# Terascale-All-sensing-Research-Studio/MOV-SLAM

Hardware: AMD Instinct MI355X
Metric: local-BA iterations/sec (50 KF x 20k MapPoint window) (higher is better)
Workload: dtype f64; 1 GPU; LocalBundleAdjustment 50 KF + 10 fixed x 20000 MapPoints, E=110510 mono edges, Huber on, 10 LM iterations (cfg3, seed 1003); one window per GPU; parallelism=1 window

## Files before the change

### mov-slam_amd/csrc/coarse_level.h

```cpp
#pragma once
#include <hip/hip_runtime.h>

#include <type_traits>

#include "device_math.h"
#include "device_types.h"
#include "handoff.h"

namespace movba {

#ifndef MOVBA_COARSE_EXTRAPOLATE
#define MOVBA_COARSE_EXTRAPOLATE 1
#endif

template <int kT, int kNC, int kPA>
__device__ __forceinline__ void coarse_build(const DevWindow &w, const PcgParams &pp, int trial, double lambda, double *sm, bool extrapolate)
{
    double *Ac = sm;
    double *gj = Ac + kNC * kNC;
    int &s_bad = *reinterpret_cast<int *>(gj + 9 * kNC + 2);
    const int tid = threadIdx.x;
    const int nf = w.nfree;
#ifdef MOVBA_CLOCK_STAMP
    unsigned long long cst_last = __builtin_amdgcn_s_memtime();
#define COARSE_STAMP(k) do { const unsigned long long _t = __builtin_amdgcn_s_memtime(); if (tid == 0) w.ctrl->dbg_seg2[k] += _t - cst_last; cst_last = _t; } while (0)
#else
#define COARSE_STAMP(k) do { } while (0)
#endif
    const double *part = w.part, *part_ = part;
    double *blocks = w.blocks_c;
    if (tid == 0) s_bad = 0;
    for (int idx = tid; idx < kNC * kNC; idx += kT) Ac[idx] = 0.0;

    const int ndiag = nf * 36;
    for (int idx = tid; idx < w.n_multi * 36; idx += kT) {
        const int m = idx / 36, k = idx - m * 36, pr = w.multi_pairs[m];
        double sacc = 0.0;
        for (int itx = w.pair_item_start[pr]; itx < w.pair_item_start[pr + 1]; ++itx) sacc += part[(size_t)itx * kPartStride + k];
        blocks[pr * 36 + k] = -sacc;
    }
    for (int base = tid; base < ndiag; base += 4 * kT) {
        int k[4], hu[4], i0[4], i1[4];
        double s[4] = { 0, 0, 0, 0 }, hp[4] = { 0, 0, 0, 0 };
        int nmax = 0;
#pragma unroll
        for (int m = 0; m < 4; ++m) {
            const int idx = min(base + m * kT, ndiag - 1);
            const int pr = idx / 36;
            k[m] = idx - pr * 36;
            const int a = k[m] / 6, b = k[m] - a * 6;
            hu[m] = 42 + (a <= b ? ut6(a, b) : ut6(b, a));
            i0[m] = w.pair_item_start[pr]; i1[m] = w.pair_item_start[pr + 1];
            nmax = max(nmax, i1[m] - i0[m]);
        }
        for (int o = 0; o < nmax; o += 6) {
            double sv[4][6], hv[4][6];
#pragma unroll
            for (int m = 0; m < 4; ++m)
#pragma unroll
                for (int u = 0; u < 6; ++u) {
                    const double *src = part + (size_t)min(i0[m] + o + u, i1[m] - 1) * kPartStride;
                    sv[m][u] = src[k[m]]; hv[m][u] = src[hu[m]];
                }
#pragma unroll
            for (int m = 0; m < 4; ++m)
#pragma unroll
                for (int u = 0; u < 6; ++u) { const bool in = i0[m] + o + u < i1[m]; s[m] += in ? sv[m][u] : 0.0; hp[m] += in ? hv[m][u] : 0.0; }
        }
#pragma unroll
        for (int m = 0; m < 4; ++m) {
            const int idx = base + m * kT;
            if (idx < ndiag) blocks[idx] = (hp[m] + ((k[m] % 7 == 0) ? lambda : 0.0)) - s[m];
        }
    }
    __syncthreads();
    COARSE_STAMP(2);
    double *aggc = gj;
    if (tid < kNC / kPA) {
        const int g0 = pp.wave_row0[tid], g1 = pp.wave_row0[tid + 1];
        aggc[tid] = g0 + 0.5 * (g1 - g0 - 1); aggc[kNC / kPA + tid] = 1.0 / fmax(1.0, 0.5 * (g1 - g0));
    }
    int *tent = reinterpret_cast<int *>(gj + 9 * kNC + 8), *tij = tent + w.cblk_ptr[w.n_cblk];
    for (int q = tid; q < w.cblk_ptr[w.n_cblk]; q += kT) { tent[q] = w.cblk_ent[q]; tij[q] = w.cblk_ij[q]; }
    __syncthreads();
    const int nw = w.n_cblk * 6;
    const bool split = 2 * nw <= kT;
    auto walk = [&](int cb, int a, int part, double (&s00)[6], double (&s01)[6], double (&s10)[6], double (&s11)[6]) {
        const int g = w.cblk_g[cb], h = w.cblk_h[cb];
        const double cg = aggc[g], ch = aggc[h], ig = aggc[kNC / kPA + g], ih = aggc[kNC / kPA + h];
        int t0 = w.cblk_ptr[cb], t1 = w.cblk_ptr[cb + 1];
        if (split) {
            const int n = t1 - t0, front = min(n, (((n + 1) >> 1) + 7) & ~7);
            if (part == 0) t1 = t0 + front; else t0 += front;
        }
#pragma unroll
        for (int m = 0; m < 6; ++m) s00[m] = s01[m] = s10[m] = s11[m] = 0.0;
        for (int t = t0; t < t1; t += 8) {
            int pk[8], ij[8];
            double v[8][6];
#pragma unroll
            for (int u = 0; u < 8; ++u) { const int tt = min(t + u, t1 - 1); pk[u] = tent[tt]; ij[u] = tij[tt]; }
#pragma unroll
            for (int u = 0; u < 8; ++u) {
                const int e = pk[u];
                const double *src = (e & 1) ? part_ + (size_t)(e >> 2) * kPartStride : blocks + (size_t)(e >> 2) * 36;
                const int o0 = (e & 2) ? a : a * 6, st = (e & 2) ? 6 : 1;
#pragma unroll
                for (int m = 0; m < 6; ++m) v[u][m] = src[o0 + st * m];
            }
#pragma unroll
            for (int u = 0; u < 8; ++u) {
                const bool in = t + u < t1;
                const double sgn = in ? ((pk[u] & 1) ? -1.0 : 1.0) : 0.0;
                const double pi = ((ij[u] >> 16) - cg) * ig, pj = ((ij[u] & 0xffff) - ch) * ih;
#pragma unroll
                for (int m = 0; m < 6; ++m) {
                    const double x = sgn * v[u][m];
                    s00[m] += x; s01[m] += pj * x; s10[m] += pi * x; s11[m] += pi * pj * x;
                }
            }
        }
        return Ac + (g * kPA + a) * kNC + h * kPA;
    };
    if (split) {
        const bool active = tid < 2 * nw;
        const int half = tid >= nw, wi = tid - half * nw;
        double s00[6], s01[6], s10[6], s11[6];
        double *dst = nullptr;
        if (active) dst = walk(wi / 6, wi - (wi / 6) * 6, half, s00, s01, s10, s11);
        if (active && !half) {
#pragma unroll
            for (int m = 0; m < 6; ++m) { dst[m] = s00[m]; dst[6 + m] = s01[m]; dst[6 * kNC + m] = s10[m]; dst[6 * kNC + 6 + m] = s11[m]; }
        }
        __syncthreads();
        if (active && half) {
#pragma unroll
            for (int m = 0; m < 6; ++m) { dst[m] += s00[m]; dst[6 + m] += s01[m]; dst[6 * kNC + m] += s10[m]; dst[6 * kNC + 6 + m] += s11[m]; }
        }
    } else {
        for (int wi = tid; wi < nw; wi += kT) {
            double s00[6], s01[6], s10[6], s11[6];
            double *dst = walk(wi / 6, wi - (wi / 6) * 6, 0, s00, s01, s10, s11);
#pragma unroll
            for (int m = 0; m < 6; ++m) { dst[m] = s00[m]; dst[6 + m] = s01[m]; dst[6 * kNC + m] = s10[m]; dst[6 * kNC + 6 + m] = s11[m]; }
        }
    }
    __syncthreads();
    if (tid < kNC) {
        const int g = tid / kPA, d = (tid - g * kPA) / 6, nrows = pp.wave_row0[g + 1] - pp.wave_row0[g];
        if (nrows == 0 || (d == 1 && nrows < 2)) {
            for (int j = 0; j < kNC; ++j) { Ac[tid * kNC + j] = 0.0; Ac[j * kNC + tid] = 0.0; }
        }
    }
    __syncthreads();
    if (tid < kNC) {
        const int g = tid / kPA, d = (tid - g * kPA) / 6, nrows = pp.wave_row0[g + 1] - pp.wave_row0[g];
        if (nrows == 0 || (d == 1 && nrows < 2)) Ac[tid * kNC + tid] = 1.0;
    }
    __syncthreads();
    if (extrapolate) {
        double *prev = w.ac_prev;
        const double lam_prev = prev[kNC * kNC], trial_prev = prev[kNC * kNC + 1];
        double gamma = 0.0;
        if (trial >= 1 && trial_prev == (double)(trial - 1) && lambda != lam_prev && MOVBA_COARSE_EXTRAPOLATE) {
            gamma = (lambda * (1.0 / 3.0) - lambda) / (lambda - lam_prev);
            gamma = fmin(fmax(gamma, -1.0), 1.0 / 3.0);
            if (!isfinite(gamma)) gamma = 0.0;
        }
        constexpr int kPer = kNC * kNC / kT;
        static_assert(kPer * kT == kNC * kNC, "one pass");
        double pv[kPer];
#pragma unroll
        for (int u = 0; u < kPer; ++u) pv[u] = prev[tid + u * kT];
        __syncthreads();
#pragma unroll
        for (int u = 0; u < kPer; ++u) {
            const double a = Ac[tid + u * kT];
            prev[tid + u * kT] = a;
            if (gamma != 0.0) Ac[tid + u * kT] = a + gamma * (a - pv[u]);
        }
        if (tid == 0) { prev[kNC * kNC] = lambda; prev[kNC * kNC + 1] = (double)trial; }
        __syncthreads();
    }

    COARSE_STAMP(3);
    static_assert(kNC == 96 && kT == 512, "tile layout written for 96 x 96 on 512 threads");
    double *dsc = gj + 8 * kNC + 2;
    double *pvs = gj + 8 * kNC;
    if (tid < kNC) { const double d = Ac[tid * kNC + tid]; dsc[tid] = (d > 0.0 && isfinite(d)) ? rsqrt(d) : 0.0; if (!(d > 0.0) || !isfinite(d)) s_bad = 1; }
    __syncthreads();
    const int rg = tid >> 4, cg = tid & 15;
    double t[3][6];
#pragma unroll
    for (int r = 0; r < 3; ++r)
#pragma unroll
        for (int q = 0; q < 6; ++q) t[r][q] = Ac[(3 * rg + r) * kNC + 6 * cg + q] * dsc[3 * rg + r] * dsc[6 * cg + q];
    unsigned live = 0;
    for (int q = 0; q < kNC / 6; ++q) {
        const int nrows = pp.wave_row0[(q >> 1) + 1] - pp.wave_row0[q >> 1];
        if (!(nrows == 0 || ((q & 1) && nrows < 2))) live |= 1u << q;
    }
    __syncthreads();
    auto publish = [&](auto Ctag, int gq, int buf) {
        constexpr int C = decltype(Ctag)::value;
        constexpr int lr0 = C % 3, lr1 = (C + 1) % 3;
        const int rg0 = 2 * gq + C / 3, rg1 = 2 * gq + (C + 1) / 3;
        double *R1 = gj + buf * 4 * kNC, *C1 = R1 + kNC, *R2 = C1 + kNC, *C2 = R2 + kNC;
        if (rg == rg0) {
#pragma unroll
            for (int q = 0; q < 6; ++q) R1[6 * cg + q] = t[lr0][q] + ((cg == gq && q == C) ? 1.0 : 0.0);
        }
        if (rg == rg1) {
#pragma unroll
            for (int q = 0; q < 6; ++q) R2[6 * cg + q] = t[lr1][q];
        }
        if (cg == gq) {
#pragma unroll
            for (int r = 0; r < 3; ++r) { C1[3 * rg + r] = t[r][C] - ((rg == rg0 && r == lr0) ? 1.0 : 0.0); C2[3 * rg + r] = t[r][C + 1]; }
        }
        if (rg == rg0 && cg == gq) pvs[buf] = t[lr0][C];
    };
    int kk = live ? __builtin_ctz(live) : kNC / 6;
    if (kk < kNC / 6) publish(std::integral_constant<int, 0>{}, kk, 0);
    __syncthreads();
    bool bad = s_bad != 0;
    int buf = 0;
    auto pair_step = [&](auto Ctag, int gq) -> bool {
        constexpr int C = decltype(Ctag)::value;
        constexpr int lr1 = (C + 1) % 3;
        const int k = 6 * gq + C, rg1 = 2 * gq + (C + 1) / 3;
        const double *R1 = gj + buf * 4 * kNC, *C1 = R1 + kNC, *R2 = C1 + kNC, *C2 = R2 + kNC;
        const double p1 = pvs[buf];
        const double o12 = R1[k + 1], o21 = C1[k + 1], q22 = R2[k + 1];
        double r1[6], r2[6], c1[3], c2[3];
#pragma unroll
        for (int q = 0; q < 6; ++q) { r1[q] = R1[6 * cg + q]; r2[q] = R2[6 * cg + q]; }
#pragma unroll
        for (int r = 0; r < 3; ++r) { c1[r] = C1[3 * rg + r]; c2[r] = C2[3 * rg + r]; }
        if (!(p1 > 0.0) || !isfinite(p1)) return false;
        double ip1 = __builtin_amdgcn_rcp(p1);
        ip1 = ip1 * (2.0 - p1 * ip1);
        ip1 = ip1 * (2.0 - p1 * ip1);
        const double s12 = o12 * ip1;
        const double p2 = q22 - o21 * s12;
        if (!(p2 > 0.0) || !isfinite(p2)) return false;
        double ip2 = __builtin_amdgcn_rcp(p2);
        ip2 = ip2 * (2.0 - p2 * ip2);
        ip2 = ip2 * (2.0 - p2 * ip2);
#pragma unroll
        for (int q = 0; q < 6; ++q) {
            r1[q] *= ip1;
            r2[q] = ((r2[q] - o21 * r1[q]) + ((cg == gq && q == C + 1) ? 1.0 : 0.0)) * ip2;
        }
#pragma unroll
        for (int r = 0; r < 3; ++r) c2[r] = (c2[r] - c1[r] * s12) - ((rg == rg1 && r == lr1) ? 1.0 : 0.0);
#pragma unroll
        for (int r = 0; r < 3; ++r)
#pragma unroll
            for (int q = 0; q < 6; ++q) { t[r][q] -= c1[r] * r1[q]; t[r][q] -= c2[r] * r2[q]; }
        return true;
    };
    while (kk < kNC / 6 && !bad) {
        const unsigned later = kk < 31 ? (live & ~((2u << kk) - 1u)) : 0u;
        const int next = later ? __builtin_ctz(later) : kNC / 6;
        if (!pair_step(std::integral_constant<int, 0>{}, kk)) { bad = true; break; }
        publish(std::integral_constant<int, 2>{}, kk, buf ^ 1);
        __syncthreads(); buf ^= 1;
        if (!pair_step(std::integral_constant<int, 2>{}, kk)) { bad = true; break; }
        publish(std::integral_constant<int, 4>{}, kk, buf ^ 1);
        __syncthreads(); buf ^= 1;
        if (!pair_step(std::integral_constant<int, 4>{}, kk)) { bad = true; break; }
        if (next < kNC / 6) publish(std::integral_constant<int, 0>{}, next, buf ^ 1);
        __syncthreads(); buf ^= 1;
        kk = next;
    }
    if (bad && tid == 0) s_bad = 1;
    __syncthreads();
    COARSE_STAMP(4);
    float *dst = w.aci + (size_t)(trial & 1) * kNC * kNC;
#pragma unroll
    for (int r = 0; r < 3; ++r)
#pragma unroll
        for (int q = 0; q < 6; ++q) dst[(3 * rg + r) * kNC + 6 * cg + q] = (float)(t[r][q] * dsc[3 * rg + r] * dsc[6 * cg + q]);
    __syncthreads();
    if (tid == 0) w.aci_tag[trial & 1] = s_bad ? -1 : trial;
    COARSE_STAMP(5);
}

}
```

Before: 9360 LM iterations/s.

## Block the coarse Gauss-Jordan inverse into 16-wide panels with f64 MFMA updates

Replaces the 2-column-at-a-time Gauss-Jordan inversion of the 96x96 coarse matrix, which issued a barrier after every pivot pair, with a panel-blocked version. Each 16-column panel is factored in registers by three waves using readlane broadcasts. The trailing update then runs as 16x16 tiles through f64 MFMA, reading double-buffered padded panel images stored in place of A_c. This cuts the barrier count from about 48 to about 12 and moves the rank updates onto matrix cores. In exchange it adds shared-memory image traffic, and the panel liveness test and sign conventions have to stay numerically equivalent to the old version.

```diff
diff --git a/mov-slam_amd/csrc/coarse_level.h b/mov-slam_amd/csrc/coarse_level.h
--- a/mov-slam_amd/csrc/coarse_level.h
+++ b/mov-slam_amd/csrc/coarse_level.h
@@ -1,7 +1,5 @@
 #pragma once
 #include <hip/hip_runtime.h>
-
-#include <type_traits>
 
 #include "device_math.h"
 #include "device_types.h"
@@ -185,103 +183,128 @@
 
     COARSE_STAMP(3);
     static_assert(kNC == 96 && kT == 512, "tile layout written for 96 x 96 on 512 threads");
+    constexpr int kPB = 16, kNP = kNC / kPB, kPL = kPB + 1;
+    constexpr int kTilesPerWave = (kNP * kNP + kT / 64 - 1) / (kT / 64);
+    static_assert(2 * 2 * kNC * kPL <= kNC * kNC, "two pairs of panel images in the place of A_c");
+    typedef double dbl4 __attribute__((ext_vector_type(4)));
     double *dsc = gj + 8 * kNC + 2;
-    double *pvs = gj + 8 * kNC;
     if (tid < kNC) { const double d = Ac[tid * kNC + tid]; dsc[tid] = (d > 0.0 && isfinite(d)) ? rsqrt(d) : 0.0; if (!(d > 0.0) || !isfinite(d)) s_bad = 1; }
     __syncthreads();
-    const int rg = tid >> 4, cg = tid & 15;
-    double t[3][6];
-#pragma unroll
-    for (int r = 0; r < 3; ++r)
-#pragma unroll
-        for (int q = 0; q < 6; ++q) t[r][q] = Ac[(3 * rg + r) * kNC + 6 * cg + q] * dsc[3 * rg + r] * dsc[6 * cg + q];
+    const int ln = tid & 63, li = ln & 15, lk = ln >> 4;
+    const int wv = __builtin_amdgcn_readfirstlane(tid >> 6);
+    dbl4 acc[kTilesPerWave];
+#pragma unroll
+    for (int u = 0; u < kTilesPerWave; ++u) {
+        const int T = wv + 8 * u, rb = T / kNP, cb = T - rb * kNP;
+        acc[u] = dbl4{ 0.0, 0.0, 0.0, 0.0 };
+        if (T < kNP * kNP) {
+#pragma unroll
+            for (int v = 0; v < 4; ++v) {
+                const int r = kPB * rb + lk + 4 * v, q = kPB * cb + li;
+                acc[u][v] = Ac[r * kNC + q] * dsc[r] * dsc[q];
+            }
+        }
+    }
     unsigned live = 0;
     for (int q = 0; q < kNC / 6; ++q) {
         const int nrows = pp.wave_row0[(q >> 1) + 1] - pp.wave_row0[q >> 1];
         if (!(nrows == 0 || ((q & 1) && nrows < 2))) live |= 1u << q;
     }
-    __syncthreads();
-    auto publish = [&](auto Ctag, int gq, int buf) {
-        constexpr int C = decltype(Ctag)::value;
-        constexpr int lr0 = C % 3, lr1 = (C + 1) % 3;
-        const int rg0 = 2 * gq + C / 3, rg1 = 2 * gq + (C + 1) / 3;
-        double *R1 = gj + buf * 4 * kNC, *C1 = R1 + kNC, *R2 = C1 + kNC, *C2 = R2 + kNC;
-        if (rg == rg0) {
-#pragma unroll
-            for (int q = 0; q < 6; ++q) R1[6 * cg + q] = t[lr0][q] + ((cg == gq && q == C) ? 1.0 : 0.0);
-        }
-        if (rg == rg1) {
-#pragma unroll
-            for (int q = 0; q < 6; ++q) R2[6 * cg + q] = t[lr1][q];
-        }
-        if (cg == gq) {
-#pragma unroll
-            for (int r = 0; r < 3; ++r) { C1[3 * rg + r] = t[r][C] - ((rg == rg0 && r == lr0) ? 1.0 : 0.0); C2[3 * rg + r] = t[r][C + 1]; }
-        }
-        if (rg == rg0 && cg == gq) pvs[buf] = t[lr0][C];
+    unsigned plive = 0;
+    for (int P = 0; P < kNP; ++P) {
+        const int q0 = (kPB * P) / 6, q1 = (kPB * P + kPB - 1) / 6;
+        if ((live >> q0) & ((2u << (q1 - q0)) - 1u)) plive |= 1u << P;
+    }
+    __syncthreads();
+    if (s_bad) plive = 0;
+    auto image = [&](int buf) { return Ac + buf * 2 * kNC * kPL; };
+    auto store_tile = [&](double *img, int rb, const dbl4 &a) {
+#pragma unroll
+        for (int v = 0; v < 4; ++v) img[(kPB * rb + lk + 4 * v) * kPL + li] = a[v];
     };
-    int kk = live ? __builtin_ctz(live) : kNC / 6;
-    if (kk < kNC / 6) publish(std::integral_constant<int, 0>{}, kk, 0);
-    __syncthreads();
-    bool bad = s_bad != 0;
-    int buf = 0;
-    auto pair_step = [&](auto Ctag, int gq) -> bool {
-        constexpr int C = decltype(Ctag)::value;
-        constexpr int lr1 = (C + 1) % 3;
-        const int k = 6 * gq + C, rg1 = 2 * gq + (C + 1) / 3;
-        const double *R1 = gj + buf * 4 * kNC, *C1 = R1 + kNC, *R2 = C1 + kNC, *C2 = R2 + kNC;
-        const double p1 = pvs[buf];
-        const double o12 = R1[k + 1], o21 = C1[k + 1], q22 = R2[k + 1];
-        double r1[6], r2[6], c1[3], c2[3];
-#pragma unroll
-        for (int q = 0; q < 6; ++q) { r1[q] = R1[6 * cg + q]; r2[q] = R2[6 * cg + q]; }
-#pragma unroll
-        for (int r = 0; r < 3; ++r) { c1[r] = C1[3 * rg + r]; c2[r] = C2[3 * rg + r]; }
-        if (!(p1 > 0.0) || !isfinite(p1)) return false;
-        double ip1 = __builtin_amdgcn_rcp(p1);
-        ip1 = ip1 * (2.0 - p1 * ip1);
-        ip1 = ip1 * (2.0 - p1 * ip1);
-        const double s12 = o12 * ip1;
-        const double p2 = q22 - o21 * s12;
-        if (!(p2 > 0.0) || !isfinite(p2)) return false;
-        double ip2 = __builtin_amdgcn_rcp(p2);
-        ip2 = ip2 * (2.0 - p2 * ip2);
-        ip2 = ip2 * (2.0 - p2 * ip2);
-#pragma unroll
-        for (int q = 0; q < 6; ++q) {
-            r1[q] *= ip1;
-            r2[q] = ((r2[q] - o21 * r1[q]) + ((cg == gq && q == C + 1) ? 1.0 : 0.0)) * ip2;
-        }
-#pragma unroll
-        for (int r = 0; r < 3; ++r) c2[r] = (c2[r] - c1[r] * s12) - ((rg == rg1 && r == lr1) ? 1.0 : 0.0);
-#pragma unroll
-        for (int r = 0; r < 3; ++r)
-#pragma unroll
-            for (int q = 0; q < 6; ++q) { t[r][q] -= c1[r] * r1[q]; t[r][q] -= c2[r] * r2[q]; }
-        return true;
+    auto chain = [&](int P, const double *O, double *N) {
+        const int c0 = kPB * P;
+        const bool real = ln < 32;
+        const int i = real ? 32 * wv + ln : c0 + li;
+        double p[kPB];
+#pragma unroll
+        for (int c = 0; c < kPB; ++c) p[c] = O[i * kPL + c];
+        bool bad = false;
+#pragma unroll
+        for (int k = 0; k < kPB; ++k) {
+            double s[kPB];
+#pragma unroll
+            for (int c = 0; c < kPB; ++c) s[c] = readlane_f64(p[c], 32 + k);
+            const double piv = s[k];
+            bad |= !(piv > 0.0 && piv < __builtin_inf());
+            const double r0 = __builtin_amdgcn_rcp(piv);
+            const double e = __builtin_fma(-piv, r0, 1.0);
+            const double t = __builtin_fma(e, e, e);
+            const double ip = __builtin_fma(r0, t, r0);
+            const double g = (p[k] - (i == c0 + k ? 1.0 : 0.0)) * ip;
+            s[k] += 1.0;
+#pragma unroll
+            for (int c = 0; c < kPB; ++c) p[c] -= g * s[c];
+        }
+        if (real) {
+#pragma unroll
+            for (int c = 0; c < kPB; ++c) N[i * kPL + c] = p[c];
+        }
+        if (bad && ln == 0) s_bad = 1;
     };
-    while (kk < kNC / 6 && !bad) {
-        const unsigned later = kk < 31 ? (live & ~((2u << kk) - 1u)) : 0u;
-        const int next = later ? __builtin_ctz(later) : kNC / 6;
-        if (!pair_step(std::integral_constant<int, 0>{}, kk)) { bad = true; break; }
-        publish(std::integral_constant<int, 2>{}, kk, buf ^ 1);
-        __syncthreads(); buf ^= 1;
-        if (!pair_step(std::integral_constant<int, 2>{}, kk)) { bad = true; break; }
-        publish(std::integral_constant<int, 4>{}, kk, buf ^ 1);
-        __syncthreads(); buf ^= 1;
-        if (!pair_step(std::integral_constant<int, 4>{}, kk)) { bad = true; break; }
-        if (next < kNC / 6) publish(std::integral_constant<int, 0>{}, next, buf ^ 1);
-        __syncthreads(); buf ^= 1;
-        kk = next;
-    }
-    if (bad && tid == 0) s_bad = 1;
-    __syncthreads();
+    int P = plive ? __builtin_ctz(plive) : kNP, buf = 0;
+    if (P < kNP) {
+#pragma unroll
+        for (int u = 0; u < kTilesPerWave; ++u) {
+            const int T = wv + 8 * u, rb = T / kNP, cb = T - rb * kNP;
+            if (T < kNP * kNP && cb == P) store_tile(image(0), rb, acc[u]);
+        }
+    }
+    __syncthreads();
+    while (P < kNP) {
+        const unsigned later = plive & ~((2u << P) - 1u);
+        const int next = later ? __builtin_ctz(later) : kNP;
+        const double *O = image(buf), *N = O + kNC * kPL;
+        if (wv < 3) chain(P, O, image(buf) + kNC * kPL);
+        __syncthreads();
+#pragma unroll
+        for (int u = 0; u < kTilesPerWave; ++u) {
+            const int T = wv + 8 * u, rb = T / kNP, cb = T - rb * kNP;
+            if (T >= kNP * kNP) continue;
+            if (cb == P) {
+#pragma unroll
+                for (int v = 0; v < 4; ++v) acc[u][v] = N[(kPB * rb + lk + 4 * v) * kPL + li];
+            } else if (rb == P) {
+                const double sgn = cb < P ? 1.0 : -1.0;
+#pragma unroll
+                for (int v = 0; v < 4; ++v) acc[u][v] = sgn * N[(kPB * cb + li) * kPL + lk + 4 * v];
+            } else {
+                const double sgn = cb > P ? 1.0 : -1.0;
+                const double *ap = N + (kPB * rb + li) * kPL + lk, *bp = O + (kPB * cb + li) * kPL + lk;
+                double a[kPB / 4], b[kPB / 4];
+#pragma unroll
+                for (int q = 0; q < kPB / 4; ++q) { a[q] = ap[4 * q]; b[q] = sgn * bp[4 * q]; }
+#pragma unroll
+                for (int q = 0; q < kPB / 4; ++q) acc[u] = __builtin_amdgcn_mfma_f64_16x16x4f64(a[q], b[q], acc[u], 0, 0, 0);
+            }
+            if (cb == next) store_tile(image(buf ^ 1), rb, acc[u]);
+        }
+        __syncthreads();
+        buf ^= 1; P = next;
+    }
     COARSE_STAMP(4);
     float *dst = w.aci + (size_t)(trial & 1) * kNC * kNC;
 #pragma unroll
-    for (int r = 0; r < 3; ++r)
-#pragma unroll
-        for (int q = 0; q < 6; ++q) dst[(3 * rg + r) * kNC + 6 * cg + q] = (float)(t[r][q] * dsc[3 * rg + r] * dsc[6 * cg + q]);
+    for (int u = 0; u < kTilesPerWave; ++u) {
+        const int T = wv + 8 * u, rb = T / kNP, cb = T - rb * kNP;
+        if (T < kNP * kNP) {
+#pragma unroll
+            for (int v = 0; v < 4; ++v) {
+                const int r = kPB * rb + lk + 4 * v, q = kPB * cb + li;
+                dst[r * kNC + q] = (float)(acc[u][v] * dsc[r] * dsc[q]);
+            }
+        }
+    }
     __syncthreads();
     if (tid == 0) w.aci_tag[trial & 1] = s_bad ? -1 : trial;
     COARSE_STAMP(5);
```

Result: faster. 9584 LM iterations/s (median of 6 runs) (+2.4%).
